# Z1HaoC/YOLO-Dual

Hardware: AMD Instinct MI355X
Metric: images/sec at 640x640 bs=16/GPU (higher is better)
Workload: dtype bf16; 1 GPU; YOLOv5-backbone (C3+SPPF) + UNet-lite SegmentHead, fwd+bwd+SGD/EMA step, 640x640, bs=16/GPU, CE+0.5*Dice, 12 classes (BASELINE configs[1]); global_batch=16, parallelism=dp1

## Files before the change

### yolo_dual_amd/csrc/spatial.hip

```cpp
#include "common.h"
#include <stdlib.h>

static inline int sgrid(long long total) {
    long long b = (total + 255) / 256;
    if (b > 256 * 16) b = 256 * 16;
    if (b < 1) b = 1;
    return (int)b;
}

template <typename T>
__global__ __launch_bounds__(256) void maxpool_fwd_kernel(const T* __restrict__ x, int ldx, T* __restrict__ y, int ldy,
                                                          uint8_t* __restrict__ idx, int N, int Hi, int Wi, int Ho, int Wo,
                                                          int Cp, int k, int s, int p) {
    constexpr int V = ET<T>::V;
    const int cpp = Cp / V;
    const long long total = (long long)N * Ho * Wo * cpp;
    for (long long i = (long long)blockIdx.x * blockDim.x + threadIdx.x; i < total; i += (long long)gridDim.x * blockDim.x) {
        int cq = (int)(i % cpp);
        long long pix = i / cpp;
        int wo = (int)(pix % Wo);
        long long t2 = pix / Wo;
        int ho = (int)(t2 % Ho);
        int n = (int)(t2 / Ho);
        float best[V];
        int bi[V];
#pragma unroll
        for (int e = 0; e < V; ++e) { best[e] = -INFINITY; bi[e] = 0; }
        bool first = true;
        for (int ky = 0; ky < k; ++ky) {
            int ih = ho * s - p + ky;
            if ((unsigned)ih >= (unsigned)Hi) continue;
            for (int kx = 0; kx < k; ++kx) {
                int iw = wo * s - p + kx;
                if ((unsigned)iw >= (unsigned)Wi) continue;
                float v[V];
                unpack16<T>(*(const uint4*)(x + ((size_t)(n * Hi + ih) * Wi + iw) * ldx + cq * V), v);
#pragma unroll
                for (int e = 0; e < V; ++e) {
                    if (first || v[e] > best[e] || v[e] != v[e]) { best[e] = v[e]; bi[e] = ky * k + kx; }
                }
                first = false;
            }
        }
        *(uint4*)(y + (size_t)pix * ldy + cq * V) = pack16<T>(best);
        if (idx) {
#pragma unroll
            for (int e = 0; e < V; ++e) idx[(size_t)pix * Cp + cq * V + e] = (uint8_t)bi[e];
        }
    }
}

template <typename T>
__global__ __launch_bounds__(256) void maxpool_bwd_kernel(const T* __restrict__ dy, int lddy, const uint8_t* __restrict__ idx,
                                                          T* __restrict__ dx, int lddx, int accumulate, int N, int Hi, int Wi,
                                                          int Ho, int Wo, int Cp, int k, int s, int p) {
    constexpr int V = ET<T>::V;
    const int cpp = Cp / V;
    const long long total = (long long)N * Hi * Wi * cpp;
    for (long long i = (long long)blockIdx.x * blockDim.x + threadIdx.x; i < total; i += (long long)gridDim.x * blockDim.x) {
        int cq = (int)(i % cpp);
        long long pix = i / cpp;
        int iw = (int)(pix % Wi);
        long long t2 = pix / Wi;
        int ih = (int)(t2 % Hi);
        int n = (int)(t2 / Hi);
        float g[V];
#pragma unroll
        for (int e = 0; e < V; ++e) g[e] = 0.f;
        if (accumulate) unpack16<T>(*(const uint4*)(dx + (size_t)pix * lddx + cq * V), g);
        for (int ky = 0; ky < k; ++ky) {
            int nh = ih + p - ky;
            if (nh < 0 || nh % s != 0) continue;
            int ho = nh / s;
            if (ho >= Ho) continue;
            for (int kx = 0; kx < k; ++kx) {
                int nw = iw + p - kx;
                if (nw < 0 || nw % s != 0) continue;
                int wo = nw / s;
                if (wo >= Wo) continue;
                size_t op = ((size_t)(n * Ho + ho) * Wo + wo);
                float d[V];
                unpack16<T>(*(const uint4*)(dy + op * lddy + cq * V), d);
                const uint8_t* ip = idx + op * Cp + cq * V;
                int code = ky * k + kx;
#pragma unroll
                for (int e = 0; e < V; ++e) g[e] += (ip[e] == code) ? d[e] : 0.f;
            }
        }
        *(uint4*)(dx + (size_t)pix * lddx + cq * V) = pack16<T>(g);
    }
}

extern "C" int ydl_maxpool_fwd(int dtype, const void* x, int ldx, void* y, int ldy, uint8_t* idx,
                               int N, int Hi, int Wi, int Ho, int Wo, int C, int k, int s, int p, void* stream) {
    const int V = dtype == YDL_F32 ? 4 : 8;
    const int Cp = round_up(C, V);
    YDL_CHECK(x && y && ldx >= Cp && ldy >= Cp && k * k <= 255, "bad arguments");
    YDL_CHECK(aligned16(x) && aligned16(y) && ldx % V == 0 && ldy % V == 0, "16-byte alignment");
    YDL_CHECK(Ho == (Hi + 2 * p - k) / s + 1 && Wo == (Wi + 2 * p - k) / s + 1, "output size mismatch");
    hipStream_t st = (hipStream_t)stream;
    int grid = sgrid((long long)N * Ho * Wo * (Cp / V));
    if (dtype == YDL_F32) maxpool_fwd_kernel<float><<<grid, 256, 0, st>>>((const float*)x, ldx, (float*)y, ldy, idx, N, Hi, Wi, Ho, Wo, Cp, k, s, p);
    else maxpool_fwd_kernel<bf16_t><<<grid, 256, 0, st>>>((const bf16_t*)x, ldx, (bf16_t*)y, ldy, idx, N, Hi, Wi, Ho, Wo, Cp, k, s, p);
    YDL_LAUNCH_CHECK();
    return 0;
}
extern "C" int ydl_maxpool_bwd(int dtype, const void* dy, int lddy, const uint8_t* idx, void* dx, int lddx, int accumulate,
                               int N, int Hi, int Wi, int Ho, int Wo, int C, int k, int s, int p, void* stream) {
    const int V = dtype == YDL_F32 ? 4 : 8;
    const int Cp = round_up(C, V);
    YDL_CHECK(dy && dx && idx && lddy >= Cp && lddx >= Cp, "bad arguments");
    YDL_CHECK(aligned16(dy) && aligned16(dx) && lddy % V == 0 && lddx % V == 0, "16-byte alignment");
    hipStream_t st = (hipStream_t)stream;
    int grid = sgrid((long long)N * Hi * Wi * (Cp / V));
    if (dtype == YDL_F32) maxpool_bwd_kernel<float><<<grid, 256, 0, st>>>((const float*)dy, lddy, idx, (float*)dx, lddx, accumulate, N, Hi, Wi, Ho, Wo, Cp, k, s, p);
    else maxpool_bwd_kernel<bf16_t><<<grid, 256, 0, st>>>((const bf16_t*)dy, lddy, idx, (bf16_t*)dx, lddx, accumulate, N, Hi, Wi, Ho, Wo, Cp, k, s, p);
    YDL_LAUNCH_CHECK();
    return 0;
}

template <int V> struct SpCodes;
template <> struct SpCodes<8> {
    typedef uint2 W;
    __device__ static __forceinline__ W pack(const int* c) {
        return make_uint2((unsigned)c[0] | ((unsigned)c[1] << 8) | ((unsigned)c[2] << 16) | ((unsigned)c[3] << 24),
                          (unsigned)c[4] | ((unsigned)c[5] << 8) | ((unsigned)c[6] << 16) | ((unsigned)c[7] << 24));
    }
    __device__ static __forceinline__ int get(const W& w, int e) { return (int)(((e < 4 ? w.x : w.y) >> ((e & 3) * 8)) & 0xffu); }
};
template <> struct SpCodes<4> {
    typedef unsigned W;
    __device__ static __forceinline__ W pack(const int* c) {
        return (unsigned)c[0] | ((unsigned)c[1] << 8) | ((unsigned)c[2] << 16) | ((unsigned)c[3] << 24);
    }
    __device__ static __forceinline__ int get(const W& w, int e) { return (int)((w >> (e * 8)) & 0xffu); }
};
#define SP_CG 2
template <typename T>
__global__ __launch_bounds__(256) void sppf_pool_fwd_kernel(const T* __restrict__ x, int ldx, T* __restrict__ y1, T* __restrict__ y2,
                                                            T* __restrict__ y3, int ldy, uint8_t* __restrict__ i1, uint8_t* __restrict__ i2,
                                                            uint8_t* __restrict__ i3, int H, int W, int Cp, int k) {
    constexpr int V = ET<T>::V;
    extern __shared__ __attribute__((aligned(16))) unsigned char sp_smem[];
    const int HW = H * W;
    const int items = HW * SP_CG;
    uint4* cur = (uint4*)sp_smem;
    uint4* rmax = cur + items;
    typedef SpCodes<V> CW;
    typename CW::W* rkx = (typename CW::W*)(rmax + items);
    const int cpp = Cp / V;
    const int n = blockIdx.y;
    const int cq0 = blockIdx.x * SP_CG;
    const int p = k / 2;
    for (int it = threadIdx.x; it < items; it += 256) {
        const int cg = it % SP_CG, pix = it / SP_CG;
        uint4 v = make_uint4(0, 0, 0, 0);
        if (cq0 + cg < cpp) v = *(const uint4*)(x + ((size_t)n * HW + pix) * ldx + (cq0 + cg) * V);
        cur[it] = v;
    }
    __syncthreads();
    T* const ys[3] = {y1, y2, y3};
    uint8_t* const is[3] = {i1, i2, i3};
#pragma unroll
    for (int st = 0; st < 3; ++st) {
        for (int it = threadIdx.x; it < items; it += 256) {
            const int cg = it % SP_CG, pix = it / SP_CG;
            const int wo = pix % W, ho = pix / W;
            float best[V];
            int bk[V];
#pragma unroll
            for (int e = 0; e < V; ++e) { best[e] = -INFINITY; bk[e] = 0; }
            bool first = true;
            for (int kx = 0; kx < k; ++kx) {
                const int iw = wo - p + kx;
                if ((unsigned)iw >= (unsigned)W) continue;
                float v[V];
                unpack16<T>(cur[(ho * W + iw) * SP_CG + cg], v);
#pragma unroll
                for (int e = 0; e < V; ++e)
                    if (first || v[e] > best[e] || v[e] != v[e]) { best[e] = v[e]; bk[e] = kx; }
                first = false;
            }
            rmax[it] = pack16<T>(best);
            rkx[it] = CW::pack(bk);
        }
        __syncthreads();
        for (int it = threadIdx.x; it < items; it += 256) {
            const int cg = it % SP_CG, pix = it / SP_CG;
            const int wo = pix % W, ho = pix / W;
            float best[V];
            int bi[V];
#pragma unroll
            for (int e = 0; e < V; ++e) { best[e] = -INFINITY; bi[e] = 0; }
            bool first = true;
            for (int ky = 0; ky < k; ++ky) {
                const int ih = ho - p + ky;
                if ((unsigned)ih >= (unsigned)H) continue;
                const int rit = (ih * W + wo) * SP_CG + cg;
                float v[V];
                unpack16<T>(rmax[rit], v);
                const typename CW::W rk = rkx[rit];
#pragma unroll
                for (int e = 0; e < V; ++e)
                    if (first || v[e] > best[e] || v[e] != v[e]) { best[e] = v[e]; bi[e] = ky * k + CW::get(rk, e); }
                first = false;
            }
            const uint4 o = pack16<T>(best);
            if (st < 2) cur[it] = o;
            if (cq0 + cg < cpp) {
                const size_t gp = (size_t)n * HW + pix;
                *(uint4*)(ys[st] + gp * ldy + (cq0 + cg) * V) = o;
                if (is[st]) *(typename CW::W*)(is[st] + gp * Cp + (cq0 + cg) * V) = CW::pack(bi);
            }
        }
        __syncthreads();
    }
}

template <typename T>
__global__ __launch_bounds__(256) void sppf_pool_bwd_kernel(const T* __restrict__ dy1, const T* __restrict__ dy2, const T* __restrict__ dy3,
                                                            int lddy, const uint8_t* __restrict__ i1, const uint8_t* __restrict__ i2,
                                                            const uint8_t* __restrict__ i3, T* __restrict__ dx, int lddx, int accumulate,
                                                            int H, int W, int Cp, int k) {
    constexpr int V = ET<T>::V;
    extern __shared__ __attribute__((aligned(16))) unsigned char sp_smem[];
    const int HW = H * W;
    uint4* plane[2] = {(uint4*)sp_smem, (uint4*)sp_smem + (size_t)HW * SP_CG};
    typedef SpCodes<V> CW;
    typename CW::W* icode = (typename CW::W*)((uint4*)sp_smem + (size_t)2 * HW * SP_CG);
    const int cpp = Cp / V;
    const int n = blockIdx.y;
    const int cq0 = blockIdx.x * SP_CG;
    const int p = k / 2;
    const int items = HW * SP_CG;
    const T* const dys[3] = {dy3, dy2, dy1};
    const uint8_t* const is[3] = {i3, i2, i1};
    for (int it = threadIdx.x; it < items; it += 256) {
        const int cg = it % SP_CG, pix = it / SP_CG;
        uint4 v = make_uint4(0, 0, 0, 0);
        if (cq0 + cg < cpp) v = *(const uint4*)(dy3 + ((size_t)n * HW + pix) * lddy + (cq0 + cg) * V);
        plane[0][it] = v;
    }
#pragma unroll
    for (int st = 0; st < 3; ++st) {
        for (int it = threadIdx.x; it < items; it += 256) {
            const int cg = it % SP_CG, pix = it / SP_CG;
            if (cq0 + cg < cpp) icode[it] = *(const typename CW::W*)(is[st] + ((size_t)n * HW + pix) * Cp + (cq0 + cg) * V);
        }
        __syncthreads();
        const uint4* src = plane[st & 1];
        uint4* dst = plane[(st + 1) & 1];
        for (int it = threadIdx.x; it < items; it += 256) {
            const int cg = it % SP_CG, pix = it / SP_CG;
            if (cq0 + cg >= cpp) continue;
            const int iw = pix % W, ih = pix / W;
            const size_t gp = (size_t)n * HW + pix;
            float g[V];
#pragma unroll
            for (int e = 0; e < V; ++e) g[e] = 0.f;
            if (st < 2) unpack16<T>(*(const uint4*)(dys[st + 1] + gp * lddy + (cq0 + cg) * V), g);
            else if (accumulate) unpack16<T>(*(const uint4*)(dx + gp * lddx + (cq0 + cg) * V), g);
            for (int ky = 0; ky < k; ++ky) {
                const int ho = ih + p - ky;
                if (ho < 0 || ho >= H) continue;
                for (int kx = 0; kx < k; ++kx) {
                    const int wo = iw + p - kx;
                    if (wo < 0 || wo >= W) continue;
                    const int oit = (ho * W + wo) * SP_CG + cg;
                    float d[V];
                    unpack16<T>(src[oit], d);
                    const typename CW::W cw = icode[oit];
                    const int code = ky * k + kx;
#pragma unroll
                    for (int e = 0; e < V; ++e) g[e] += (CW::get(cw, e) == code) ? d[e] : 0.f;
                }
            }
            const uint4 o = pack16<T>(g);
            if (st < 2) dst[it] = o;
            else *(uint4*)(dx + gp * lddx + (cq0 + cg) * V) = o;
        }
        __syncthreads();
    }
}

static inline size_t sppf_smem(int dtype, int H, int W, bool bwd) {
    const int V = dtype == YDL_F32 ? 4 : 8;
    (void)bwd;
    return (size_t)H * W * SP_CG * (2 * 16 + V);
}
extern "C" int ydl_sppf_pool_supported(int dtype, int H, int W, int C, int k) {
    if (dtype != YDL_F32 && dtype != YDL_BF16) return 0;
    if (k < 1 || k % 2 == 0 || k * k > 255 || H < 1 || W < 1 || C < 1) return 0;
    return sppf_smem(dtype, H, W, true) <= 64 * 1024 ? 1 : 0;
}
extern "C" int ydl_sppf_pool_fwd(int dtype, const void* x, int ldx, void* y1, void* y2, void* y3, int ldy,
                                 uint8_t* idx1, uint8_t* idx2, uint8_t* idx3, int N, int H, int W, int C, int k, void* stream) {
    const int V = dtype == YDL_F32 ? 4 : 8;
    const int Cp = round_up(C, V);
    YDL_CHECK(ydl_sppf_pool_supported(dtype, H, W, C, k), "plane too large for the LDS-resident form (query ydl_sppf_pool_supported)");
    YDL_CHECK(x && y1 && y2 && y3 && ldx >= Cp && ldy >= Cp && N >= 1, "bad arguments");
    YDL_CHECK((idx1 == nullptr) == (idx2 == nullptr) && (idx2 == nullptr) == (idx3 == nullptr), "the three index planes come together");
    YDL_CHECK(aligned16(x) && aligned16(y1) && aligned16(y2) && aligned16(y3) && ldx % V == 0 && ldy % V == 0, "16-byte alignment");
    hipStream_t st = (hipStream_t)stream;
    const dim3 grid((Cp / V + SP_CG - 1) / SP_CG, N);
    const size_t smem = sppf_smem(dtype, H, W, false);
    if (dtype == YDL_F32) sppf_pool_fwd_kernel<float><<<grid, 256, smem, st>>>((const float*)x, ldx, (float*)y1, (float*)y2, (float*)y3, ldy, idx1, idx2, idx3, H, W, Cp, k);
    else sppf_pool_fwd_kernel<bf16_t><<<grid, 256, smem, st>>>((const bf16_t*)x, ldx, (bf16_t*)y1, (bf16_t*)y2, (bf16_t*)y3, ldy, idx1, idx2, idx3, H, W, Cp, k);
    YDL_LAUNCH_CHECK();
    return 0;
}
extern "C" int ydl_sppf_pool_bwd(int dtype, const void* dy1, const void* dy2, const void* dy3, int lddy, const uint8_t* idx1,
                                 const uint8_t* idx2, const uint8_t* idx3, void* dx, int lddx, int accumulate,
                                 int N, int H, int W, int C, int k, void* stream) {
    const int V = dtype == YDL_F32 ? 4 : 8;
    const int Cp = round_up(C, V);
    YDL_CHECK(ydl_sppf_pool_supported(dtype, H, W, C, k), "plane too large for the LDS-resident form (query ydl_sppf_pool_supported)");
    YDL_CHECK(dy1 && dy2 && dy3 && idx1 && idx2 && idx3 && dx && lddy >= Cp && lddx >= Cp && N >= 1, "bad arguments");
    YDL_CHECK(aligned16(dy1) && aligned16(dy2) && aligned16(dy3) && aligned16(dx) && lddy % V == 0 && lddx % V == 0, "16-byte alignment");
    hipStream_t st = (hipStream_t)stream;
    const dim3 grid((Cp / V + SP_CG - 1) / SP_CG, N);
    const size_t smem = sppf_smem(dtype, H, W, true);
    if (dtype == YDL_F32) sppf_pool_bwd_kernel<float><<<grid, 256, smem, st>>>((const float*)dy1, (const float*)dy2, (const float*)dy3, lddy, idx1, idx2, idx3, (float*)dx, lddx, accumulate, H, W, Cp, k);
    else sppf_pool_bwd_kernel<bf16_t><<<grid, 256, smem, st>>>((const bf16_t*)dy1, (const bf16_t*)dy2, (const bf16_t*)dy3, lddy, idx1, idx2, idx3, (bf16_t*)dx, lddx, accumulate, H, W, Cp, k);
    YDL_LAUNCH_CHECK();
    return 0;
}

struct Lin { int i0, i1; float w0, w1; };

__device__ __forceinline__ Lin lin_src(int dst, float scale, int in, bool align) {
    Lin L;
    float src;
    if (align) {
        src = __fmul_rn(scale, (float)dst);
    } else {
        src = __fsub_rn(__fmul_rn(scale, __fadd_rn((float)dst, 0.5f)), 0.5f);
        if (src < 0.f) src = 0.f;
    }
    L.i0 = (int)src;
    if (L.i0 > in - 1) L.i0 = in - 1;
    L.i1 = L.i0 + (L.i0 < in - 1 ? 1 : 0);
    L.w1 = __fsub_rn(src, (float)L.i0);
    L.w0 = __fsub_rn(1.f, L.w1);
    return L;
}
__device__ __forceinline__ int near_src(int dst, float scale, int in) {
    int v = (int)floorf(__fmul_rn((float)dst, scale));
    return v < in - 1 ? v : in - 1;
}

template <typename T>
__global__ __launch_bounds__(256) void resize_fwd_kernel(int mode, const T* __restrict__ x, int ldx, T* __restrict__ y, int ldy,
                                                         int N, int Hi, int Wi, int Ho, int Wo, int Cp, float sh, float sw) {
    constexpr int V = ET<T>::V;
    const int cpp = Cp / V;
    const long long total = (long long)N * Ho * Wo * cpp;
    for (long long i = (long long)blockIdx.x * blockDim.x + threadIdx.x; i < total; i += (long long)gridDim.x * blockDim.x) {
        int cq = (int)(i % cpp);
        long long pix = i / cpp;
        int wo = (int)(pix % Wo);
        long long t2 = pix / Wo;
        int ho = (int)(t2 % Ho);
        int n = (int)(t2 / Ho);
        const T* xb = x + (size_t)n * Hi * Wi * ldx + cq * V;
        float o[V];
        if (mode == 0) {
            int ih = near_src(ho, sh, Hi), iw = near_src(wo, sw, Wi);
            *(uint4*)(y + (size_t)pix * ldy + cq * V) = *(const uint4*)(xb + ((size_t)ih * Wi + iw) * ldx);
            continue;
        }
        Lin lh = lin_src(ho, sh, Hi, mode == 2), lw = lin_src(wo, sw, Wi, mode == 2);
        float v00[V], v01[V], v10[V], v11[V];
        unpack16<T>(*(const uint4*)(xb + ((size_t)lh.i0 * Wi + lw.i0) * ldx), v00);
        unpack16<T>(*(const uint4*)(xb + ((size_t)lh.i0 * Wi + lw.i1) * ldx), v01);
        unpack16<T>(*(const uint4*)(xb + ((size_t)lh.i1 * Wi + lw.i0) * ldx), v10);
        unpack16<T>(*(const uint4*)(xb + ((size_t)lh.i1 * Wi + lw.i1) * ldx), v11);
#pragma unroll
        for (int e = 0; e < V; ++e)
            o[e] = lh.w0 * (lw.w0 * v00[e] + lw.w1 * v01[e]) + lh.w1 * (lw.w0 * v10[e] + lw.w1 * v11[e]);
        *(uint4*)(y + (size_t)pix * ldy + cq * V) = pack16<T>(o);
    }
}

__device__ __forceinline__ void cand_range(int i, int in, int out, float scale, int mode, int& lo, int& hi) {
    float inv = scale > 0.f ? 1.0f / scale : (float)out;
    float a = ((float)i - 1.5f) * inv - 2.f, b = ((float)i + 1.5f) * inv + 2.f;
    if (mode == 0) { a = (float)i * inv - 2.f; b = ((float)i + 1.f) * inv + 2.f; }
    lo = a < 0.f ? 0 : (int)a;
    hi = b > (float)(out - 1) ? out - 1 : (int)b;
    if (i == in - 1) hi = out - 1;
    if (i == 0) lo = 0;
}

template <typename T>
__global__ __launch_bounds__(256) void resize_bwd_kernel(int mode, const T* __restrict__ dy, int lddy, T* __restrict__ dx, int lddx,
                                                         int accumulate, int N, int Hi, int Wi, int Ho, int Wo, int Cp, float sh, float sw) {
    constexpr int V = ET<T>::V;
    const int cpp = Cp / V;
    const long long total = (long long)N * Hi * Wi * cpp;
    for (long long i = (long long)blockIdx.x * blockDim.x + threadIdx.x; i < total; i += (long long)gridDim.x * blockDim.x) {
        int cq = (int)(i % cpp);
        long long pix = i / cpp;
        int iw = (int)(pix % Wi);
        long long t2 = pix / Wi;
        int ih = (int)(t2 % Hi);
        int n = (int)(t2 / Hi);
        float g[V];
#pragma unroll
        for (int e = 0; e < V; ++e) g[e] = 0.f;
        if (accumulate) unpack16<T>(*(const uint4*)(dx + (size_t)pix * lddx + cq * V), g);
        int hlo, hhi, wlo, whi;
        cand_range(ih, Hi, Ho, sh, mode, hlo, hhi);
        cand_range(iw, Wi, Wo, sw, mode, wlo, whi);
        const T* db = dy + (size_t)n * Ho * Wo * lddy + cq * V;
        for (int ho = hlo; ho <= hhi; ++ho) {
            float wh;
            if (mode == 0) wh = near_src(ho, sh, Hi) == ih ? 1.f : 0.f;
            else { Lin l = lin_src(ho, sh, Hi, mode == 2); wh = (l.i0 == ih ? l.w0 : 0.f) + (l.i1 == ih ? l.w1 : 0.f); }
            if (wh == 0.f) continue;
            for (int wo = wlo; wo <= whi; ++wo) {
                float ww;
                if (mode == 0) ww = near_src(wo, sw, Wi) == iw ? 1.f : 0.f;
                else { Lin l = lin_src(wo, sw, Wi, mode == 2); ww = (l.i0 == iw ? l.w0 : 0.f) + (l.i1 == iw ? l.w1 : 0.f); }
                if (ww == 0.f) continue;
                float d[V];
                unpack16<T>(*(const uint4*)(db + ((size_t)ho * Wo + wo) * lddy), d);
                float wgt = wh * ww;
#pragma unroll
                for (int e = 0; e < V; ++e) g[e] += wgt * d[e];
            }
        }
        *(uint4*)(dx + (size_t)pix * lddx + cq * V) = pack16<T>(g);
    }
}

template <typename T, int S>
__global__ __launch_bounds__(256) void resize_bwd_int_kernel(const T* __restrict__ dy, int lddy, T* __restrict__ dx, int lddx, int accumulate,
                                                             int N, int Hi, int Wi, int Cp, float sh, float sw) {
    constexpr int V = ET<T>::V;
    constexpr int NC = 2 * S;
    const int Ho = Hi * S, Wo = Wi * S;
    const int cpp = Cp / V;
    const long long total = (long long)N * Hi * Wi * cpp;
    for (long long i = (long long)blockIdx.x * blockDim.x + threadIdx.x; i < total; i += (long long)gridDim.x * blockDim.x) {
        const int cq = (int)(i % cpp);
        const long long pix = i / cpp;
        const int iw = (int)(pix % Wi);
        const long long t2 = pix / Wi;
        const int ih = (int)(t2 % Hi);
        const int n = (int)(t2 / Hi);
        float g[V];
#pragma unroll
        for (int e = 0; e < V; ++e) g[e] = 0.f;
        if (accumulate) unpack16<T>(*(const uint4*)(dx + (size_t)pix * lddx + cq * V), g);
        float wwv[NC];
#pragma unroll
        for (int b = 0; b < NC; ++b) {
            const int wo = S * iw - S / 2 + b;
            float ww = 0.f;
            if ((unsigned)wo < (unsigned)Wo) { const Lin l = lin_src(wo, sw, Wi, false); ww = (l.i0 == iw ? l.w0 : 0.f) + (l.i1 == iw ? l.w1 : 0.f); }
            wwv[b] = ww;
        }
        const T* db = dy + (size_t)n * Ho * Wo * lddy + cq * V;
#pragma unroll
        for (int a = 0; a < NC; ++a) {
            const int ho = S * ih - S / 2 + a;
            if ((unsigned)ho >= (unsigned)Ho) continue;
            const Lin l = lin_src(ho, sh, Hi, false);
            const float wh = (l.i0 == ih ? l.w0 : 0.f) + (l.i1 == ih ? l.w1 : 0.f);
            if (wh == 0.f) continue;
#pragma unroll
            for (int b = 0; b < NC; ++b) {
                const int wo = S * iw - S / 2 + b;
                if (wwv[b] == 0.f) continue;
                float d[V];
                unpack16<T>(*(const uint4*)(db + ((size_t)ho * Wo + wo) * lddy), d);
                const float wgt = wh * wwv[b];
#pragma unroll
                for (int e = 0; e < V; ++e) g[e] += wgt * d[e];
            }
        }
        *(uint4*)(dx + (size_t)pix * lddx + cq * V) = pack16<T>(g);
    }
}

template <typename T, bool ACC>
__global__ __launch_bounds__(256) void resize_acc_sums_kernel(int mode, const T* __restrict__ x, int ldx, T* __restrict__ y, int ldy,
                                                              int Hi, int Wi, int Ho, int Wo, int Cp, float sh, float sw,
                                                              int nrows, float* __restrict__ sums, int sums_ld) {
    constexpr int V = ET<T>::V;
    const int cpp = Cp / V;
    const int cpb = cpp < 256 ? cpp : 256;
    const int R = 256 / cpb;
    const int cq = threadIdx.x % cpb, pl = threadIdx.x / cpb;
    const int chunk = blockIdx.y * 256 + cq;
    const bool live = pl < R && chunk < cpp;
    const int c0 = chunk * V;
    float s1[V], s2[V];
#pragma unroll
    for (int e = 0; e < V; ++e) { s1[e] = 0.f; s2[e] = 0.f; }
    if (live) {
        for (int row = blockIdx.x; row < nrows; row += gridDim.x) {
            const int n = row / Ho, ho = row - n * Ho;
            const T* xb = x + (size_t)n * Hi * Wi * ldx + c0;
            T* yrow = y + (size_t)row * Wo * ldy + c0;
            Lin lh;
            int ihn = 0;
            if (mode == 0) ihn = near_src(ho, sh, Hi);
            else lh = lin_src(ho, sh, Hi, mode == 2);
            const T* r0 = xb + (size_t)(mode == 0 ? ihn : lh.i0) * Wi * ldx;
            const T* r1 = xb + (size_t)(mode == 0 ? ihn : lh.i1) * Wi * ldx;
            for (int wo = pl; wo < Wo; wo += R) {
                float o[V], yv[V];
                if (mode == 0) {
                    unpack16<T>(*(const uint4*)(r0 + (size_t)near_src(wo, sw, Wi) * ldx), o);
                } else {
                    const Lin lw = lin_src(wo, sw, Wi, mode == 2);
                    float v00[V], v01[V], v10[V], v11[V];
                    unpack16<T>(*(const uint4*)(r0 + (size_t)lw.i0 * ldx), v00);
                    unpack16<T>(*(const uint4*)(r0 + (size_t)lw.i1 * ldx), v01);
                    unpack16<T>(*(const uint4*)(r1 + (size_t)lw.i0 * ldx), v10);
                    unpack16<T>(*(const uint4*)(r1 + (size_t)lw.i1 * ldx), v11);
#pragma unroll
                    for (int e = 0; e < V; ++e)
                        o[e] = lh.w0 * (lw.w0 * v00[e] + lw.w1 * v01[e]) + lh.w1 * (lw.w0 * v10[e] + lw.w1 * v11[e]);
                }
                T* yp = yrow + (size_t)wo * ldy;
                if constexpr (ACC) {
                    unpack16<T>(*(const uint4*)yp, yv);
#pragma unroll
                    for (int e = 0; e < V; ++e) {
                        const float v = yv[e] + o[e];
                        yv[e] = v;
                        s1[e] += v;
                        s2[e] = fmaf(v, v, s2[e]);
                    }
                    *(uint4*)yp = pack16<T>(yv);
                } else {
                    *(uint4*)yp = pack16<T>(o);
                }
            }
        }
    }
    if (!ACC || sums == nullptr) return;
    __shared__ float red[256 * 2 * 8];
#pragma unroll
    for (int e = 0; e < V; ++e) {
        red[(threadIdx.x * 2 + 0) * V + e] = live ? s1[e] : 0.f;
        red[(threadIdx.x * 2 + 1) * V + e] = live ? s2[e] : 0.f;
    }
    __syncthreads();
    if (threadIdx.x < cpb && chunk < cpp) {
        float* dst = sums + (size_t)(blockIdx.x & (YDL_BN_REPLICAS - 1)) * 2 * sums_ld;
#pragma unroll
        for (int e = 0; e < V; ++e) {
            float a = 0.f, b = 0.f;
            for (int l = 0; l < R; ++l) {
                const int tt = l * cpb + threadIdx.x;
                a += red[(tt * 2 + 0) * V + e];
                b += red[(tt * 2 + 1) * V + e];
            }
            atomicAdd(dst + c0 + e, a);
            atomicAdd(dst + sums_ld + c0 + e, b);
        }
    }
}

struct Cub { int i[4]; float c[4]; };

__device__ __forceinline__ float cubic_c1(float x) {
    return __fadd_rn(__fmul_rn(__fmul_rn(__fsub_rn(__fmul_rn(1.25f, x), 2.25f), x), x), 1.f);
}
__device__ __forceinline__ float cubic_c2(float x) {
    return __fsub_rn(__fmul_rn(__fadd_rn(__fmul_rn(__fsub_rn(__fmul_rn(-0.75f, x), -3.75f), x), -6.f), x), -3.f);
}
__device__ __forceinline__ Cub cub_src(int dst, float scale, int in, bool align) {
    Cub Q;
    const float src = align ? __fmul_rn(scale, (float)dst) : __fsub_rn(__fmul_rn(scale, __fadd_rn((float)dst, 0.5f)), 0.5f);
    const float fl = floorf(src);
    const float t = __fsub_rn(src, fl);
    const float u = __fsub_rn(1.f, t);
    const int i0 = (int)fl;
    Q.c[0] = cubic_c2(__fadd_rn(t, 1.f));
    Q.c[1] = cubic_c1(t);
    Q.c[2] = cubic_c1(u);
    Q.c[3] = cubic_c2(__fadd_rn(u, 1.f));
#pragma unroll
    for (int j = 0; j < 4; ++j) {
        int v = i0 - 1 + j;
        v = v < 0 ? 0 : v;
        Q.i[j] = v > in - 1 ? in - 1 : v;
    }
    return Q;
}
__device__ __forceinline__ float cub_weight(const Cub& Q, int i) {
    float w = 0.f;
#pragma unroll
    for (int j = 0; j < 4; ++j) w = __fadd_rn(w, Q.i[j] == i ? Q.c[j] : 0.f);
    return w;
}

template <typename T>
__global__ __launch_bounds__(256) void bicubic_fwd_kernel(int align, const T* __restrict__ x, int ldx, T* __restrict__ y, int ldy,
                                                          int Hi, int Wi, int Ho, int Wo, int Cp, float sh, float sw, int nrows) {
    constexpr int V = ET<T>::V;
    const int cpp = Cp / V;
    const int cpb = cpp < 256 ? cpp : 256;
    const int R = 256 / cpb;
    const int cq = threadIdx.x % cpb, pl = threadIdx.x / cpb;
    const int chunk = blockIdx.y * 256 + cq;
    if (!(pl < R && chunk < cpp)) return;
    const int c0 = chunk * V;
    for (int row = blockIdx.x; row < nrows; row += gridDim.x) {
        const int n = row / Ho, ho = row - n * Ho;
        const T* xb = x + (size_t)n * Hi * Wi * ldx + c0;
        T* yrow = y + (size_t)row * Wo * ldy + c0;
        const Cub qh = cub_src(ho, sh, Hi, align != 0);
        for (int wo = pl; wo < Wo; wo += R) {
            const Cub qw = cub_src(wo, sw, Wi, align != 0);
            float o[V];
#pragma unroll
            for (int e = 0; e < V; ++e) o[e] = 0.f;
#pragma unroll
            for (int a = 0; a < 4; ++a) {
                const T* r = xb + (size_t)qh.i[a] * Wi * ldx;
                float rs[V];
// ... 613 lines not shown
```

Baseline: 2699 images/sec.

## Rewrite bf16 SPPF max-pool with order-preserving integer keys and retuned launch

For bf16, the SPPF forward now converts values to monotone 32-bit integer keys with the kernel offset packed into the low bits. Each window max, together with its argmax, then becomes a single integer max, and the per-element compare-and-select logic goes away. If any NaN is seen the block falls back to the float path. The change also cuts channel groups per block to 1 and sizes the thread count to the plane with up to 512 threads, which gives more blocks and better occupancy. It also swizzles the block index across 8 groups, and the backward pass gains precomputed loop bounds in place of per-iteration bounds checks.

```diff
diff --git a/yolo_dual_amd/csrc/spatial.hip b/yolo_dual_amd/csrc/spatial.hip
--- a/yolo_dual_amd/csrc/spatial.hip
+++ b/yolo_dual_amd/csrc/spatial.hip
@@ -135,36 +135,46 @@
     }
     __device__ static __forceinline__ int get(const W& w, int e) { return (int)((w >> (e * 8)) & 0xffu); }
 };
-#define SP_CG 2
-template <typename T>
-__global__ __launch_bounds__(256) void sppf_pool_fwd_kernel(const T* __restrict__ x, int ldx, T* __restrict__ y1, T* __restrict__ y2,
-                                                            T* __restrict__ y3, int ldy, uint8_t* __restrict__ i1, uint8_t* __restrict__ i2,
-                                                            uint8_t* __restrict__ i3, int H, int W, int Cp, int k) {
-    constexpr int V = ET<T>::V;
-    extern __shared__ __attribute__((aligned(16))) unsigned char sp_smem[];
+template <typename T> struct SpFwd { static constexpr int CG = 2, MAXT = 256; };
+template <> struct SpFwd<bf16_t> { static constexpr int CG = 1, MAXT = 512; };
+#define SP_BWD_CG 1
+#define SP_BWD_MAXT 512
+
+__device__ __forceinline__ void sp_block(int& cq, int& n) {
+    const int nb = gridDim.x * gridDim.y;
+    int b = blockIdx.x + gridDim.x * blockIdx.y;
+    if (nb % 8 == 0) b = (b % 8) * (nb / 8) + b / 8;
+    cq = b % (int)gridDim.x;
+    n = b / (int)gridDim.x;
+}
+
+template <typename T, int CG>
+__device__ __forceinline__ void sppf_fwd_float(unsigned char* smem, const T* __restrict__ x, int ldx, T* const* ys, int ldy,
+                                               uint8_t* const* is, int H, int W, int Cp, int k) {
+    constexpr int V = ET<T>::V;
     const int HW = H * W;
-    const int items = HW * SP_CG;
-    uint4* cur = (uint4*)sp_smem;
+    const int items = HW * CG;
+    const int nt = blockDim.x;
+    uint4* cur = (uint4*)smem;
     uint4* rmax = cur + items;
     typedef SpCodes<V> CW;
     typename CW::W* rkx = (typename CW::W*)(rmax + items);
     const int cpp = Cp / V;
-    const int n = blockIdx.y;
-    const int cq0 = blockIdx.x * SP_CG;
+    int cq0, n;
+    sp_block(cq0, n);
+    cq0 *= CG;
     const int p = k / 2;
-    for (int it = threadIdx.x; it < items; it += 256) {
-        const int cg = it % SP_CG, pix = it / SP_CG;
+    for (int it = threadIdx.x; it < items; it += nt) {
+        const int cg = it % CG, pix = it / CG;
         uint4 v = make_uint4(0, 0, 0, 0);
         if (cq0 + cg < cpp) v = *(const uint4*)(x + ((size_t)n * HW + pix) * ldx + (cq0 + cg) * V);
         cur[it] = v;
     }
     __syncthreads();
-    T* const ys[3] = {y1, y2, y3};
-    uint8_t* const is[3] = {i1, i2, i3};
 #pragma unroll
     for (int st = 0; st < 3; ++st) {
-        for (int it = threadIdx.x; it < items; it += 256) {
-            const int cg = it % SP_CG, pix = it / SP_CG;
+        for (int it = threadIdx.x; it < items; it += nt) {
+            const int cg = it % CG, pix = it / CG;
             const int wo = pix % W, ho = pix / W;
             float best[V];
             int bk[V];
@@ -175,7 +185,7 @@
                 const int iw = wo - p + kx;
                 if ((unsigned)iw >= (unsigned)W) continue;
                 float v[V];
-                unpack16<T>(cur[(ho * W + iw) * SP_CG + cg], v);
+                unpack16<T>(cur[(ho * W + iw) * CG + cg], v);
 #pragma unroll
                 for (int e = 0; e < V; ++e)
                     if (first || v[e] > best[e] || v[e] != v[e]) { best[e] = v[e]; bk[e] = kx; }
@@ -185,8 +195,8 @@
             rkx[it] = CW::pack(bk);
         }
         __syncthreads();
-        for (int it = threadIdx.x; it < items; it += 256) {
-            const int cg = it % SP_CG, pix = it / SP_CG;
+        for (int it = threadIdx.x; it < items; it += nt) {
+            const int cg = it % CG, pix = it / CG;
             const int wo = pix % W, ho = pix / W;
             float best[V];
             int bi[V];
@@ -196,7 +206,7 @@
             for (int ky = 0; ky < k; ++ky) {
                 const int ih = ho - p + ky;
                 if ((unsigned)ih >= (unsigned)H) continue;
-                const int rit = (ih * W + wo) * SP_CG + cg;
+                const int rit = (ih * W + wo) * CG + cg;
                 float v[V];
                 unpack16<T>(rmax[rit], v);
                 const typename CW::W rk = rkx[rit];
@@ -217,41 +227,153 @@
     }
 }
 
-template <typename T>
-__global__ __launch_bounds__(256) void sppf_pool_bwd_kernel(const T* __restrict__ dy1, const T* __restrict__ dy2, const T* __restrict__ dy3,
-                                                            int lddy, const uint8_t* __restrict__ i1, const uint8_t* __restrict__ i2,
-                                                            const uint8_t* __restrict__ i3, T* __restrict__ dx, int lddx, int accumulate,
-                                                            int H, int W, int Cp, int k) {
-    constexpr int V = ET<T>::V;
+__device__ __forceinline__ unsigned sp_key(unsigned b) {
+    const unsigned mag = b & 0x7fffu;
+    return (((b & 0x8000u) ? 0x8000u - mag : 0x8000u + mag) << 16) | (b == 0x8000u ? 1u : 0u);
+}
+__device__ __forceinline__ unsigned sp_unkey(unsigned w) {
+    const int s = (int)(w >> 16) - 0x8000;
+    return (s >= 0 ? (unsigned)s : 0x8000u | (unsigned)-s) | ((w & 1u) << 15);
+}
+template <int CG>
+__device__ __forceinline__ bool sppf_fwd_keys(unsigned char* smem, const bf16_t* __restrict__ x, int ldx, bf16_t* const* ys, int ldy,
+                                              uint8_t* const* is, int H, int W, int Cp, int k) {
+    const int HW = H * W;
+    const int items = HW * CG;
+    const int nt = blockDim.x;
+    uint4* pl = (uint4*)smem;
+    uint4* rw = pl + 2 * items;
+    const int cpp = Cp / 8;
+    int cq0, n;
+    sp_block(cq0, n);
+    cq0 *= CG;
+    const int p = k / 2;
+    int nan = 0;
+    for (int it = threadIdx.x; it < items; it += nt) {
+        const int cg = it % CG, pix = it / CG;
+        uint4 v = make_uint4(0, 0, 0, 0);
+        if (cq0 + cg < cpp) v = *(const uint4*)(x + ((size_t)n * HW + pix) * ldx + (cq0 + cg) * 8);
+        const unsigned h[4] = {v.x, v.y, v.z, v.w};
+        unsigned w[8];
+#pragma unroll
+        for (int j = 0; j < 4; ++j) {
+            const unsigned lo = h[j] & 0xffffu, hi = h[j] >> 16;
+            nan |= ((lo & 0x7fffu) > 0x7f80u) | ((hi & 0x7fffu) > 0x7f80u);
+            w[2 * j] = sp_key(lo);
+            w[2 * j + 1] = sp_key(hi);
+        }
+        pl[it] = make_uint4(w[0], w[1], w[2], w[3]);
+        pl[items + it] = make_uint4(w[4], w[5], w[6], w[7]);
+    }
+    if (__syncthreads_or(nan)) return false;
+#pragma unroll
+    for (int st = 0; st < 3; ++st) {
+        for (int it = threadIdx.x; it < items; it += nt) {
+            const int cg = it % CG, pix = it / CG;
+            const int wo = pix % W, ho = pix / W;
+            const int lo = p - wo > 0 ? p - wo : 0, hi = W + p - wo < k ? W + p - wo : k;
+            const int base = (ho * W + wo - p) * CG + cg;
+            unsigned b[8] = {0, 0, 0, 0, 0, 0, 0, 0};
+            for (int kx = lo; kx < hi; ++kx) {
+                const uint4 a = pl[base + kx * CG], c = pl[items + base + kx * CG];
+                const unsigned t = (unsigned)(15 - kx) << 4;
+                b[0] = max(b[0], a.x | t); b[1] = max(b[1], a.y | t); b[2] = max(b[2], a.z | t); b[3] = max(b[3], a.w | t);
+                b[4] = max(b[4], c.x | t); b[5] = max(b[5], c.y | t); b[6] = max(b[6], c.z | t); b[7] = max(b[7], c.w | t);
+            }
+            rw[it] = make_uint4(b[0], b[1], b[2], b[3]);
+            rw[items + it] = make_uint4(b[4], b[5], b[6], b[7]);
+        }
+        __syncthreads();
+        for (int it = threadIdx.x; it < items; it += nt) {
+            const int cg = it % CG, pix = it / CG;
+            const int wo = pix % W, ho = pix / W;
+            const int lo = p - ho > 0 ? p - ho : 0, hi = H + p - ho < k ? H + p - ho : k;
+            const int base = ((ho - p) * W + wo) * CG + cg;
+            unsigned b[8] = {0, 0, 0, 0, 0, 0, 0, 0};
+            for (int ky = lo; ky < hi; ++ky) {
+                const uint4 a = rw[base + ky * W * CG], c = rw[items + base + ky * W * CG];
+                const unsigned t = (unsigned)(15 - ky) << 8;
+                b[0] = max(b[0], a.x | t); b[1] = max(b[1], a.y | t); b[2] = max(b[2], a.z | t); b[3] = max(b[3], a.w | t);
+                b[4] = max(b[4], c.x | t); b[5] = max(b[5], c.y | t); b[6] = max(b[6], c.z | t); b[7] = max(b[7], c.w | t);
+            }
+            if (st < 2) {
+                pl[it] = make_uint4(b[0] & 0xffff0001u, b[1] & 0xffff0001u, b[2] & 0xffff0001u, b[3] & 0xffff0001u);
+                pl[items + it] = make_uint4(b[4] & 0xffff0001u, b[5] & 0xffff0001u, b[6] & 0xffff0001u, b[7] & 0xffff0001u);
+            }
+            if (cq0 + cg < cpp) {
+                const size_t gp = (size_t)n * HW + pix;
+                uint4 o;
+                o.x = sp_unkey(b[0]) | (sp_unkey(b[1]) << 16);
+                o.y = sp_unkey(b[2]) | (sp_unkey(b[3]) << 16);
+                o.z = sp_unkey(b[4]) | (sp_unkey(b[5]) << 16);
+                o.w = sp_unkey(b[6]) | (sp_unkey(b[7]) << 16);
+                *(uint4*)(ys[st] + gp * ldy + (cq0 + cg) * 8) = o;
+                if (is[st]) {
+                    int code[8];
+#pragma unroll
+                    for (int e = 0; e < 8; ++e) code[e] = (15 - (int)((b[e] >> 8) & 15u)) * k + 15 - (int)((b[e] >> 4) & 15u);
+                    *(uint2*)(is[st] + gp * Cp + (cq0 + cg) * 8) = SpCodes<8>::pack(code);
+                }
+            }
+        }
+        __syncthreads();
+    }
+    return true;
+}
+
+template <typename T>
+__global__ __launch_bounds__(SpFwd<T>::MAXT) void sppf_pool_fwd_kernel(const T* __restrict__ x, int ldx, T* __restrict__ y1,
+                                                                       T* __restrict__ y2, T* __restrict__ y3, int ldy,
+                                                                       uint8_t* __restrict__ i1, uint8_t* __restrict__ i2,
+                                                                       uint8_t* __restrict__ i3, int H, int W, int Cp, int k) {
+    extern __shared__ __attribute__((aligned(16))) unsigned char sp_smem[];
+    T* const ys[3] = {y1, y2, y3};
+    uint8_t* const is[3] = {i1, i2, i3};
+    if constexpr (sizeof(T) == 2) {
+        if (sppf_fwd_keys<SpFwd<T>::CG>(sp_smem, x, ldx, ys, ldy, is, H, W, Cp, k)) return;
+    }
+    sppf_fwd_float<T, SpFwd<T>::CG>(sp_smem, x, ldx, ys, ldy, is, H, W, Cp, k);
+}
+
+template <typename T>
+__global__ __launch_bounds__(SP_BWD_MAXT) void sppf_pool_bwd_kernel(const T* __restrict__ dy1, const T* __restrict__ dy2,
+                                                                    const T* __restrict__ dy3, int lddy, const uint8_t* __restrict__ i1,
+                                                                    const uint8_t* __restrict__ i2, const uint8_t* __restrict__ i3,
+                                                                    T* __restrict__ dx, int lddx, int accumulate, int H, int W, int Cp,
+                                                                    int k) {
+    constexpr int V = ET<T>::V;
+    constexpr int CG = SP_BWD_CG;
     extern __shared__ __attribute__((aligned(16))) unsigned char sp_smem[];
     const int HW = H * W;
-    uint4* plane[2] = {(uint4*)sp_smem, (uint4*)sp_smem + (size_t)HW * SP_CG};
+    const int nt = blockDim.x;
+    uint4* plane[2] = {(uint4*)sp_smem, (uint4*)sp_smem + (size_t)HW * CG};
     typedef SpCodes<V> CW;
-    typename CW::W* icode = (typename CW::W*)((uint4*)sp_smem + (size_t)2 * HW * SP_CG);
+    typename CW::W* icode = (typename CW::W*)((uint4*)sp_smem + (size_t)2 * HW * CG);
     const int cpp = Cp / V;
-    const int n = blockIdx.y;
-    const int cq0 = blockIdx.x * SP_CG;
+    int cq0, n;
+    sp_block(cq0, n);
+    cq0 *= CG;
     const int p = k / 2;
-    const int items = HW * SP_CG;
+    const int items = HW * CG;
     const T* const dys[3] = {dy3, dy2, dy1};
     const uint8_t* const is[3] = {i3, i2, i1};
-    for (int it = threadIdx.x; it < items; it += 256) {
-        const int cg = it % SP_CG, pix = it / SP_CG;
+    for (int it = threadIdx.x; it < items; it += nt) {
+        const int cg = it % CG, pix = it / CG;
         uint4 v = make_uint4(0, 0, 0, 0);
         if (cq0 + cg < cpp) v = *(const uint4*)(dy3 + ((size_t)n * HW + pix) * lddy + (cq0 + cg) * V);
         plane[0][it] = v;
     }
 #pragma unroll
     for (int st = 0; st < 3; ++st) {
-        for (int it = threadIdx.x; it < items; it += 256) {
-            const int cg = it % SP_CG, pix = it / SP_CG;
+        for (int it = threadIdx.x; it < items; it += nt) {
+            const int cg = it % CG, pix = it / CG;
             if (cq0 + cg < cpp) icode[it] = *(const typename CW::W*)(is[st] + ((size_t)n * HW + pix) * Cp + (cq0 + cg) * V);
         }
         __syncthreads();
         const uint4* src = plane[st & 1];
         uint4* dst = plane[(st + 1) & 1];
-        for (int it = threadIdx.x; it < items; it += 256) {
-            const int cg = it % SP_CG, pix = it / SP_CG;
+        for (int it = threadIdx.x; it < items; it += nt) {
+            const int cg = it % CG, pix = it / CG;
             if (cq0 + cg >= cpp) continue;
             const int iw = pix % W, ih = pix / W;
             const size_t gp = (size_t)n * HW + pix;
@@ -260,13 +382,12 @@
             for (int e = 0; e < V; ++e) g[e] = 0.f;
             if (st < 2) unpack16<T>(*(const uint4*)(dys[st + 1] + gp * lddy + (cq0 + cg) * V), g);
             else if (accumulate) unpack16<T>(*(const uint4*)(dx + gp * lddx + (cq0 + cg) * V), g);
-            for (int ky = 0; ky < k; ++ky) {
-                const int ho = ih + p - ky;
-                if (ho < 0 || ho >= H) continue;
-                for (int kx = 0; kx < k; ++kx) {
-                    const int wo = iw + p - kx;
-                    if (wo < 0 || wo >= W) continue;
-                    const int oit = (ho * W + wo) * SP_CG + cg;
+            const int ky0 = ih + p - H + 1 > 0 ? ih + p - H + 1 : 0, ky1 = ih + p + 1 < k ? ih + p + 1 : k;
+            const int kx0 = iw + p - W + 1 > 0 ? iw + p - W + 1 : 0, kx1 = iw + p + 1 < k ? iw + p + 1 : k;
+            for (int ky = ky0; ky < ky1; ++ky) {
+                const int orow = ((ih + p - ky) * W + iw + p) * CG + cg;
+                for (int kx = kx0; kx < kx1; ++kx) {
+                    const int oit = orow - kx * CG;
                     float d[V];
                     unpack16<T>(src[oit], d);
                     const typename CW::W cw = icode[oit];
@@ -283,15 +404,15 @@
     }
 }
 
-static inline size_t sppf_smem(int dtype, int H, int W, bool bwd) {
-    const int V = dtype == YDL_F32 ? 4 : 8;
-    (void)bwd;
-    return (size_t)H * W * SP_CG * (2 * 16 + V);
-}
 extern "C" int ydl_sppf_pool_supported(int dtype, int H, int W, int C, int k) {
     if (dtype != YDL_F32 && dtype != YDL_BF16) return 0;
     if (k < 1 || k % 2 == 0 || k * k > 255 || H < 1 || W < 1 || C < 1) return 0;
-    return sppf_smem(dtype, H, W, true) <= 64 * 1024 ? 1 : 0;
+    const int V = dtype == YDL_F32 ? 4 : 8;
+    return (size_t)H * W * 2 * (2 * 16 + V) <= 64 * 1024 ? 1 : 0;
+}
+static inline int sppf_threads(int items, int maxt) {
+    const int t = round_up(items, 64);
+    return t < maxt ? t : maxt;
 }
 extern "C" int ydl_sppf_pool_fwd(int dtype, const void* x, int ldx, void* y1, void* y2, void* y3, int ldy,
                                  uint8_t* idx1, uint8_t* idx2, uint8_t* idx3, int N, int H, int W, int C, int k, void* stream) {
@@ -302,10 +423,17 @@
     YDL_CHECK((idx1 == nullptr) == (idx2 == nullptr) && (idx2 == nullptr) == (idx3 == nullptr), "the three index planes come together");
     YDL_CHECK(aligned16(x) && aligned16(y1) && aligned16(y2) && aligned16(y3) && ldx % V == 0 && ldy % V == 0, "16-byte alignment");
     hipStream_t st = (hipStream_t)stream;
-    const dim3 grid((Cp / V + SP_CG - 1) / SP_CG, N);
-    const size_t smem = sppf_smem(dtype, H, W, false);
-    if (dtype == YDL_F32) sppf_pool_fwd_kernel<float><<<grid, 256, smem, st>>>((const float*)x, ldx, (float*)y1, (float*)y2, (float*)y3, ldy, idx1, idx2, idx3, H, W, Cp, k);
-    else sppf_pool_fwd_kernel<bf16_t><<<grid, 256, smem, st>>>((const bf16_t*)x, ldx, (bf16_t*)y1, (bf16_t*)y2, (bf16_t*)y3, ldy, idx1, idx2, idx3, H, W, Cp, k);
+    if (dtype == YDL_F32) {
+        constexpr int CG = SpFwd<float>::CG;
+        const dim3 grid((Cp / V + CG - 1) / CG, N);
+        const size_t smem = (size_t)H * W * CG * (2 * 16 + V);
+        sppf_pool_fwd_kernel<float><<<grid, sppf_threads(H * W * CG, SpFwd<float>::MAXT), smem, st>>>((const float*)x, ldx, (float*)y1, (float*)y2, (float*)y3, ldy, idx1, idx2, idx3, H, W, Cp, k);
+    } else {
+        constexpr int CG = SpFwd<bf16_t>::CG;
+        const dim3 grid((Cp / V + CG - 1) / CG, N);
+        const size_t smem = (size_t)H * W * CG * 64;
+        sppf_pool_fwd_kernel<bf16_t><<<grid, sppf_threads(H * W * CG, SpFwd<bf16_t>::MAXT), smem, st>>>((const bf16_t*)x, ldx, (bf16_t*)y1, (bf16_t*)y2, (bf16_t*)y3, ldy, idx1, idx2, idx3, H, W, Cp, k);
+    }
     YDL_LAUNCH_CHECK();
     return 0;
 }
@@ -318,10 +446,11 @@
     YDL_CHECK(dy1 && dy2 && dy3 && idx1 && idx2 && idx3 && dx && lddy >= Cp && lddx >= Cp && N >= 1, "bad arguments");
     YDL_CHECK(aligned16(dy1) && aligned16(dy2) && aligned16(dy3) && aligned16(dx) && lddy % V == 0 && lddx % V == 0, "16-byte alignment");
     hipStream_t st = (hipStream_t)stream;
-    const dim3 grid((Cp / V + SP_CG - 1) / SP_CG, N);
-    const size_t smem = sppf_smem(dtype, H, W, true);
-    if (dtype == YDL_F32) sppf_pool_bwd_kernel<float><<<grid, 256, smem, st>>>((const float*)dy1, (const float*)dy2, (const float*)dy3, lddy, idx1, idx2, idx3, (float*)dx, lddx, accumulate, H, W, Cp, k);
-    else sppf_pool_bwd_kernel<bf16_t><<<grid, 256, smem, st>>>((const bf16_t*)dy1, (const bf16_t*)dy2, (const bf16_t*)dy3, lddy, idx1, idx2, idx3, (bf16_t*)dx, lddx, accumulate, H, W, Cp, k);
+    const dim3 grid((Cp / V + SP_BWD_CG - 1) / SP_BWD_CG, N);
+    const size_t smem = (size_t)H * W * SP_BWD_CG * (2 * 16 + V);
+    const int nt = sppf_threads(H * W * SP_BWD_CG, SP_BWD_MAXT);
+    if (dtype == YDL_F32) sppf_pool_bwd_kernel<float><<<grid, nt, smem, st>>>((const float*)dy1, (const float*)dy2, (const float*)dy3, lddy, idx1, idx2, idx3, (float*)dx, lddx, accumulate, H, W, Cp, k);
+    else sppf_pool_bwd_kernel<bf16_t><<<grid, nt, smem, st>>>((const bf16_t*)dy1, (const bf16_t*)dy2, (const bf16_t*)dy3, lddy, idx1, idx2, idx3, (bf16_t*)dx, lddx, accumulate, H, W, Cp, k);
     YDL_LAUNCH_CHECK();
     return 0;
 }
```

Result: no change. 2722 images/sec (median of 6 runs) (+0.9%).
